# RocketFlash/EmbeddingNet

Measured on AMD Instinct MI355X. Metric: images/sec training (ResNet18, 224², triplet batch-hard) @ 1/2/4/8 GPU, higher is better.
Workload: dtype f32; 1 GPU; resnet18 224x224x3 synthetic U[0,1), 107-class P x K sampling, local batch 32x4=128 (139 resident batches cycled), E=256, margin 0.5, mining 'hardest' per local batch, radam, fp32 tensors (conv products on 16-bit MFMA from operand splits, fp32 accumulate: 3x3 stride-1 convs and their weight gradients, and the ResNets' other convs where both operands' ranges are known: two fp16 pieces + a per-tenso; global_batch=128, parallelism=dp1, active_triplets_min=192, dead_steps=0, resident_batches=139, step_mode=eager, mining=hardest

## Files before the change

### embeddingnet_amd/csrc/nn_kernels.hip

```cpp
#include "common.h"
#include "multi_tensor.h"
#include "gemm_engine.h"
#include <stdlib.h>
#include "../../include/embnet.h"

namespace embnet {

__device__ __forceinline__ float4 ld4(const float* p, long i) { return reinterpret_cast<const float4*>(p)[i]; }
__device__ __forceinline__ void st4(float* p, long i, float4 v) { reinterpret_cast<float4*>(p)[i] = v; }
__device__ __forceinline__ void add4(float4& a, float4 v) { a.x += v.x; a.y += v.y; a.z += v.z; a.w += v.w; }
__device__ __forceinline__ float4 affine4(float4 v, float4 sc, float4 sh) {
  return make_float4(fmaf(v.x, sc.x, sh.x), fmaf(v.y, sc.y, sh.y), fmaf(v.z, sc.z, sh.z), fmaf(v.w, sc.w, sh.w));
}
__device__ __forceinline__ float4 act_apply4(int act, float4 v) {
  return make_float4(act_apply(act, v.x), act_apply(act, v.y), act_apply(act, v.z), act_apply(act, v.w));
}
__device__ __forceinline__ float4 act_grad4(int act, float4 xv, float4 sc, float4 sh, float4 dz) {
  return make_float4(act_grad(act, fmaf(xv.x, sc.x, sh.x), dz.x), act_grad(act, fmaf(xv.y, sc.y, sh.y), dz.y),
                     act_grad(act, fmaf(xv.z, sc.z, sh.z), dz.z), act_grad(act, fmaf(xv.w, sc.w, sh.w), dz.w));
}
__device__ __forceinline__ float4 relu_mask4(float4 x, float4 v) {
  return make_float4(x.x > 0.f ? v.x : 0.f, x.y > 0.f ? v.y : 0.f, x.z > 0.f ? v.z : 0.f, x.w > 0.f ? v.w : 0.f);
}

// ... 30 lines not shown
  DropArg d{seed, seed_add, 0u, 1.f};
  if (rate > 0.f) { d.thr = (uint32_t)((double)rate * 4294967296.0); d.keep_scale = 1.f / (1.f - rate); }
  return d;
}
static DropArg no_drop() { return drop_arg(0.f, 0, nullptr); }
__device__ __forceinline__ uint64_t drop_seed(const DropArg& d) { return d.seed + (d.seed_add ? *d.seed_add : 0ull); }
__device__ __forceinline__ float4 drop4(const DropArg& d, uint64_t seed, long i4, float4 v) {
  const uint64_t e = (uint64_t)i4 * 4;
  v.x = rng_u32(seed, e, 1) >= d.thr ? v.x * d.keep_scale : 0.f;
  v.y = rng_u32(seed, e + 1, 1) >= d.thr ? v.y * d.keep_scale : 0.f;
  v.z = rng_u32(seed, e + 2, 1) >= d.thr ? v.z * d.keep_scale : 0.f;
  v.w = rng_u32(seed, e + 3, 1) >= d.thr ? v.w * d.keep_scale : 0.f;
  return v;
}

struct ColGeom { int cl, rl, blocks, rows_per_block; };

static ColGeom col_geom(long m, int c) {
  ColGeom g;
  int cl = 1; while (cl < c && cl < 256) cl <<= 1;
  g.cl = cl; g.rl = 256 / cl;
  long blocks = (m + (long)g.rl * 16 - 1) / ((long)g.rl * 16);
  if (blocks < 512) {
    blocks = (m + (long)g.rl * 4 - 1) / ((long)g.rl * 4);
    if (blocks > 512) blocks = 512;
  }
  if (blocks > 2048) blocks = 2048;
  if (blocks < 1) blocks = 1;
  g.blocks = (int)blocks;
  g.rows_per_block = (int)((m + blocks - 1) / blocks);
  return g;
}

template <class F>
__device__ __forceinline__ void col_reduce2(long m, int c, ColGeom g, float* __restrict__ partial, F f) {
  __shared__ float sh[2][256];
  const int ci = threadIdx.x % g.cl, ri = threadIdx.x / g.cl;
  const long r0 = (long)blockIdx.x * g.rows_per_block;
  const long r1 = min(r0 + g.rows_per_block, m);
  for (int c0 = 0; c0 < c; c0 += g.cl) {
    const int col = c0 + ci;
    float a = 0.f, b = 0.f;
    if (col < c)
      for (long r = r0 + ri; r < r1; r += g.rl) f(r, col, a, b);
    sh[0][threadIdx.x] = a; sh[1][threadIdx.x] = b;
// ... 49 lines not shown
}
__device__ __forceinline__ float tensor_bound(const float* __restrict__ bound, int c) {
  float m = 0.f;
  for (int i = threadIdx.x; i < c; i += 256) m = fmaxf(m, bound[i]);
  return block_max256<true>(m);
}

__global__ __launch_bounds__(256) void bn_stats_kernel(const float* __restrict__ x, long m, int c, ColGeom g,
                                                       float* __restrict__ partial) {
  col_reduce2(m, c, g, partial, [&](long r, int col, float& a, float& b) {
    const float v = x[r * c + col]; a += v; b = fmaf(v, v, b);
  });
}

struct NoPrep { __device__ __forceinline__ int operator()(int) const { return 0; } };
template <bool MAX3 = false, class P, class F>
__device__ __forceinline__ void col_reduce2_v4p(long m, int c4, ColGeom g, float* __restrict__ partial, P prep, F f,
                                                float* __restrict__ pmax = nullptr) {
  __shared__ float4 sh4[MAX3 ? 3 : 2][256];
  const int ci = threadIdx.x % g.cl, ri = threadIdx.x / g.cl;
  const long r0 = (long)blockIdx.x * g.rows_per_block;
  const long r1 = min(r0 + g.rows_per_block, m);
  for (int q0 = 0; q0 < c4; q0 += g.cl) {
    const int q = q0 + ci;
    float4 a = make_float4(0.f, 0.f, 0.f, 0.f), b = a, mx = a;
    if (q < c4) {
      const auto k = prep(q);
      long r = r0 + ri;
      const long rl = g.rl;
      if constexpr (MAX3) {
        for (; r + 3 * rl < r1; r += 4 * rl) { f(r, q, k, a, b, mx); f(r + rl, q, k, a, b, mx); f(r + 2 * rl, q, k, a, b, mx); f(r + 3 * rl, q, k, a, b, mx); }
        for (; r < r1; r += rl) f(r, q, k, a, b, mx);
      } else {
        for (; r + 3 * rl < r1; r += 4 * rl) { f(r, q, k, a, b); f(r + rl, q, k, a, b); f(r + 2 * rl, q, k, a, b); f(r + 3 * rl, q, k, a, b); }
        for (; r < r1; r += rl) f(r, q, k, a, b);
      }
    }
    int groups = g.rl;
    if (g.cl < 64) {
      for (int o = g.cl; o < 64; o <<= 1) {
        a.x += __shfl_xor(a.x, o, 64); a.y += __shfl_xor(a.y, o, 64); a.z += __shfl_xor(a.z, o, 64); a.w += __shfl_xor(a.w, o, 64);
        b.x += __shfl_xor(b.x, o, 64); b.y += __shfl_xor(b.y, o, 64); b.z += __shfl_xor(b.z, o, 64); b.w += __shfl_xor(b.w, o, 64);
        if constexpr (MAX3) {
          mx.x = fmaxf(mx.x, __shfl_xor(mx.x, o, 64)); mx.y = fmaxf(mx.y, __shfl_xor(mx.y, o, 64));
          mx.z = fmaxf(mx.z, __shfl_xor(mx.z, o, 64)); mx.w = fmaxf(mx.w, __shfl_xor(mx.w, o, 64));
        }
      }
      groups = 4;
      if ((threadIdx.x & 63) < g.cl) {
        sh4[0][(threadIdx.x >> 6) * g.cl + ci] = a; sh4[1][(threadIdx.x >> 6) * g.cl + ci] = b;
        if constexpr (MAX3) sh4[2][(threadIdx.x >> 6) * g.cl + ci] = mx;
      }
    } else {
      sh4[0][threadIdx.x] = a; sh4[1][threadIdx.x] = b;
      if constexpr (MAX3) sh4[2][threadIdx.x] = mx;
    }
    __syncthreads();
    if (ri == 0 && q < c4) {
      a = sh4[0][ci]; b = sh4[1][ci];
      if constexpr (MAX3) mx = sh4[2][ci];
      for (int k = 1; k < groups; ++k) {
        const float4 oa = sh4[0][k * g.cl + ci], ob = sh4[1][k * g.cl + ci];
        add4(a, oa); add4(b, ob);
        if constexpr (MAX3) {
          const float4 om = sh4[2][k * g.cl + ci];
          mx.x = fmaxf(mx.x, om.x); mx.y = fmaxf(mx.y, om.y); mx.z = fmaxf(mx.z, om.z); mx.w = fmaxf(mx.w, om.w);
        }
      }
      st4(partial + ((long)blockIdx.x * 2 + 0) * c4 * 4, q, a);
      st4(partial + ((long)blockIdx.x * 2 + 1) * c4 * 4, q, b);
      if constexpr (MAX3) st4(pmax + (long)blockIdx.x * c4 * 4, q, mx);
    }
    __syncthreads();
  }
}
template <class F>
__device__ __forceinline__ void col_reduce2_v4(long m, int c4, ColGeom g, float* __restrict__ partial, F f) {
  col_reduce2_v4p(m, c4, g, partial, NoPrep(), [&](long r, int q, int, float4& a, float4& b) { f(r, q, a, b); });
}

__global__ __launch_bounds__(256) void bn_stats4_kernel(const float* __restrict__ x, long m, int c4, ColGeom g,
                                                        float* __restrict__ partial) {
  col_reduce2_v4(m, c4, g, partial, [&](long r, int q, float4& a, float4& b) {
    const float4 v = ld4(x, r * c4 + q);
    add4(a, v);
    b.x = fmaf(v.x, v.x, b.x); b.y = fmaf(v.y, v.y, b.y); b.z = fmaf(v.z, v.z, b.z); b.w = fmaf(v.w, v.w, b.w);
  });
}

__device__ __forceinline__ float4 ld_pad4(const float* __restrict__ x, long p, int c, int q) {
  const float* s = x + p * c + 4 * q;
  if (c == 3) return make_float4(s[0], s[1], s[2], 0.f);
  const int live = c - 4 * q;
  return make_float4(s[0], live > 1 ? s[1] : 0.f, live > 2 ? s[2] : 0.f, live > 3 ? s[3] : 0.f);
}
__global__ __launch_bounds__(256) void bn_stats_pad4_kernel(const float* __restrict__ x, long m, int c, int c4, ColGeom g,
                                                            float* __restrict__ partial) {
  col_reduce2_v4(m, c4, g, partial, [&](long r, int q, float4& a, float4& b) {
    const float4 v = ld_pad4(x, r, c, q);
    add4(a, v);
    b.x = fmaf(v.x, v.x, b.x); b.y = fmaf(v.y, v.y, b.y); b.z = fmaf(v.z, v.z, b.z); b.w = fmaf(v.w, v.w, b.w);
  });
}

__global__ __launch_bounds__(256) void bn_bwd_reduce4_kernel(const float* __restrict__ dy, const float* __restrict__ x,
                                                             long m, int c4, ColGeom g, const float* __restrict__ mean,
                                                             const float* __restrict__ rstd, const float* __restrict__ scale,
                                                             const float* __restrict__ shift, int relu,
                                                             float* __restrict__ partial, const DropArg drop, float* __restrict__ pmax) {
  const uint64_t dseed = drop.thr ? drop_seed(drop) : 0ull;
  auto prep = [&](int q) { return bn_consts<false>(q, scale, shift, mean, rstd, nullptr, nullptr, 1); };
  auto body = [&](long r, int q, const BnConsts& k, float4& a, float4& b, float4& mx) {
    const float4 xv = ld4(x, r * c4 + q);
    float4 dz = ld4(dy, r * c4 + q);
    if (drop.thr) dz = drop4(drop, dseed, r * c4 + q, dz);
    if (relu) dz = act_grad4(relu, xv, k.sc, k.sh, dz);
    bn_sums4(a, b, dz, xv, k.mu, k.rs);
    mx.x = fmaxf(mx.x, fabsf(dz.x)); mx.y = fmaxf(mx.y, fabsf(dz.y)); mx.z = fmaxf(mx.z, fabsf(dz.z)); mx.w = fmaxf(mx.w, fabsf(dz.w));
  };
  if (pmax) col_reduce2_v4p<true>(m, c4, g, partial, prep, body, pmax);
  else col_reduce2_v4p(m, c4, g, partial, prep, [&](long r, int q, const BnConsts& k, float4& a, float4& b) {
    float4 mx = make_float4(0.f, 0.f, 0.f, 0.f); body(r, q, k, a, b, mx);
  });
}

template <int MODE, class DZ>
__device__ __forceinline__ void bn_bwd_apply4_body(DZ dz_of, const float* __restrict__ x, long total4, int c4, float inv_m,
                                                   const float* __restrict__ mean, const float* __restrict__ rstd,
                                                   const float* __restrict__ scale, const float* __restrict__ shift,
                                                   const float* __restrict__ dbeta, const float* __restrict__ dgamma, int relu,
                                                   int training, const float* __restrict__ dx_add, float* __restrict__ dx,
                                                   unsigned short* __restrict__ dx_planes, uint32_t* __restrict__ range_slot,
                                                   const float* __restrict__ dx_bound, const uint32_t* __restrict__ add_range) {
  const long stride = (long)gridDim.x * 256;
  const bool fixed = stride % c4 == 0;
  const float4 z4 = make_float4(0.f, 0.f, 0.f, 0.f);
  BnConsts k{z4, z4, z4, z4, z4, z4};
// ... 75 lines not shown
                     __fadd_rn(__fmul_rn(g.z, inv), dy.z), __fadd_rn(__fmul_rn(g.w, inv), dy.w));
}
__device__ __forceinline__ float4 gate4(float4 dy, const float* __restrict__ gate, long idx) {
  if (!gate) return dy;
  const float4 s = ld4(gate, idx);
  return make_float4(__fmul_rn(dy.x, s.x), __fmul_rn(dy.y, s.y), __fmul_rn(dy.z, s.z), __fmul_rn(dy.w, s.w));
}

__global__ __launch_bounds__(256) void bn_bwd_reduce4_gap_kernel(const float* __restrict__ dy, const float* __restrict__ dpool,
                                                                 const float* __restrict__ gate, DivU dhw, float inv_hw, const float* __restrict__ x, long m,
                                                                 int c4, ColGeom g, const float* __restrict__ mean,
                                                                 const float* __restrict__ rstd, const float* __restrict__ scale,
                                                                 const float* __restrict__ shift, int relu,
                                                                 float* __restrict__ partial) {
  col_reduce2_v4p(m, c4, g, partial, [&](int q) { return bn_consts<false>(q, scale, shift, mean, rstd, nullptr, nullptr, 1); },
                  [&](long r, int q, const BnConsts& k, float4& a, float4& b) {
    const float4 xv = ld4(x, r * c4 + q);
    const long nq = (long)divu((uint32_t)r, dhw) * c4 + q;
    const float4 gp = ld4(dpool, nq);
    float4 dz = add_pool4(gate4(ld4(dy, r * c4 + q), gate, nq), gp, inv_hw);
    if (relu) dz = act_grad4(relu, xv, k.sc, k.sh, dz);
    bn_sums4(a, b, dz, xv, k.mu, k.rs);
  });
}

__global__ __launch_bounds__(256) void bn_bwd_apply4_gap_kernel(const float* __restrict__ dy, const float* __restrict__ dpool,
                                                                const float* __restrict__ gate, DivU dhwc4, float inv_hw, const float* __restrict__ x,
                                                                long total4, int c4, float inv_m, const float* __restrict__ mean,
                                                                const float* __restrict__ rstd, const float* __restrict__ scale,
                                                                const float* __restrict__ shift, const float* __restrict__ dbeta,
                                                                const float* __restrict__ dgamma, int relu, float* __restrict__ dx) {
  bn_bwd_apply4_body<0>([&](long i) {
    const long nq = (long)divu((uint32_t)i, dhwc4) * c4 + (int)(i % c4);
    const float4 gp = ld4(dpool, nq);
    return add_pool4(gate4(ld4(dy, i), gate, nq), gp, inv_hw);
// ... 89 lines not shown
  b = wave_sum(b); g = wave_sum(g);
  if (lane == 0) { dbeta[col] = (float)b; dgamma[col] = (float)g; }
}

__global__ __launch_bounds__(256) void bn_bwd_apply_inrelu4_kernel(const float* __restrict__ dy, const float* __restrict__ x,
                                                                   long m, int c4, ColGeom g, float inv_m,
                                                                   const float* __restrict__ mean, const float* __restrict__ rstd,
                                                                   const float* __restrict__ scale, const float* __restrict__ shift,
                                                                   const float* __restrict__ dbeta, const float* __restrict__ dgamma,
                                                                   int relu, int training, float* __restrict__ dz_out,
                                                                   float* __restrict__ partial, const DropArg drop,
                                                                   uint32_t* __restrict__ range_slot) {
  const uint64_t dseed = drop.thr ? drop_seed(drop) : 0ull;
  float amax = 0.f;
  col_reduce2_v4p(m, c4, g, partial, [&](int q) { return bn_consts(q, scale, shift, mean, rstd, dbeta, dgamma, training); },
                  [&](long r, int q, const BnConsts& k, float4& a, float4&) {
    const float4 xv = ld4(x, r * c4 + q);
    float4 dz = ld4(dy, r * c4 + q);
    if (drop.thr) dz = drop4(drop, dseed, r * c4 + q, dz);
    if (relu) dz = act_grad4(relu, xv, k.sc, k.sh, dz);
    const float4 o = relu_mask4(xv, bn_dx4(dz, xv, k, inv_m, training));
    reinterpret_cast<float4*>(dz_out)[r * c4 + q] = o;
    add4(a, o);
    amax = amax4(amax, o);
  });
  if (range_slot) range_emit_block(range_slot + 1 + blockIdx.x % RANGE_PARTIALS, amax);
}

__global__ __launch_bounds__(256) void bn_finalize_kernel(const float* __restrict__ partial, int blocks, long m, int c,
                                                          const float* __restrict__ gamma, const float* __restrict__ beta,
                                                          float eps, float momentum, float* __restrict__ mean_out,
                                                          float* __restrict__ rstd_out, float* __restrict__ scale,
                                                          float* __restrict__ shift, float* __restrict__ moving_mean,
// ... 292 lines not shown
  const long i = (long)blockIdx.x * 256 + threadIdx.x;
  if (i >= total) return;
  const int col = (int)(i % c4);
  long t = i / c4;
  const int iw = (int)(t % w); t /= w;
  const int ih = (int)(t % h);
  const int b = (int)(t / h);
  st4(dx, i, pool_taps_grad4(dy, argmax, b, ih, iw, col, c4, k, stride, pad, oh, ow));
}

__global__ __launch_bounds__(256) void maxpool_relu_bwd_colsum4_kernel(
    const float* __restrict__ dy, const uint8_t* __restrict__ argmax, const float* __restrict__ y, long m, int h, int w,
    DivU dw, DivU dh, int c4, int k, int stride, int pad, int oh, int ow, ColGeom g, float* __restrict__ dz,
    float* __restrict__ partial, uint32_t* __restrict__ range_slot) {
  float amax = 0.f;
  col_reduce2_v4(m, c4, g, partial, [&](long r, int q, float4& a, float4& b) {
    const uint32_t t = divu((uint32_t)r, dw);
    const int iw = (int)((uint32_t)r - t * (uint32_t)w);
    const uint32_t img = divu(t, dh);
    const int ih = (int)(t - img * (uint32_t)h);
    const float4 v = relu_mask4(ld4(y, r * c4 + q), pool_taps_grad4(dy, argmax, (int)img, ih, iw, q, c4, k, stride, pad, oh, ow));
    st4(dz, r * c4 + q, v);
    add4(a, v);
    amax = amax4(amax, v);
  });
  if (range_slot) range_emit_block(range_slot + 1 + blockIdx.x % RANGE_PARTIALS, amax);
}

__global__ __launch_bounds__(256) void affine_act_maxpool_fwd4_kernel(
    const float* __restrict__ x, int n, int h, int w, int c4, const float* __restrict__ scale,
    const float* __restrict__ shift, int act, int k, int stride, int pad, int oh, int ow, float* __restrict__ y,
    uint8_t* __restrict__ argmax, float* __restrict__ xwin) {
  const long total = (long)n * oh * ow * c4;
  const long i = (long)blockIdx.x * 256 + threadIdx.x;
  if (i >= total) return;
  const int col = (int)(i % c4);
// ... 2 lines not shown
  const int y_o = (int)(t % oh);
  const int b = (int)(t / oh);
  const float4 sc = ld4(scale, col), sh = ld4(shift, col);
  const PoolWin win = pool_scan4(x, b, y_o, x_o, h, w, col, c4, k, stride, pad,
                                 [&](float4 v) { return act_apply4(act, affine4(v, sc, sh)); });
  if (xwin) st4(xwin, i, make_float4(win.xin[0], win.xin[1], win.xin[2], win.xin[3]));
  st4(y, i, make_float4(win.best[0], win.best[1], win.best[2], win.best[3]));
  reinterpret_cast<uint32_t*>(argmax)[i] = pack_taps(win.tap);
}

__global__ __launch_bounds__(256) void pool_bn_bwd_reduce4_kernel(
    const float* __restrict__ dy, const uint8_t* __restrict__ argmax, const float* __restrict__ x, long mp, int h, int w,
    int c4, int k, int stride, int pad, int oh, int ow, ColGeom g, const float* __restrict__ mean,
    const float* __restrict__ rstd, const float* __restrict__ scale, const float* __restrict__ shift, int act,
    const float* __restrict__ xwin, float* __restrict__ partial) {
  col_reduce2_v4(mp, c4, g, partial, [&](long r, int q, float4& a, float4& b) {
    const uint32_t am = reinterpret_cast<const uint32_t*>(argmax)[r * c4 + q];
    float4 xw4 = make_float4(0.f, 0.f, 0.f, 0.f);
    if (xwin) xw4 = ld4(xwin, r * c4 + q);
    const float xwv[4] = {xw4.x, xw4.y, xw4.z, xw4.w};
    const float4 d = ld4(dy, r * c4 + q);
    const int x_o = (int)(r % ow); const long t = r / ow;
    const int y_o = (int)(t % oh), bb = (int)(t / oh);
    const float4 sc = ld4(scale, q), sh = ld4(shift, q), mu = ld4(mean, q), rs = ld4(rstd, q);
    const float dd[4] = {d.x, d.y, d.z, d.w}, scv[4] = {sc.x, sc.y, sc.z, sc.w}, shv[4] = {sh.x, sh.y, sh.z, sh.w};
    const float muv[4] = {mu.x, mu.y, mu.z, mu.w}, rsv[4] = {rs.x, rs.y, rs.z, rs.w};
    float av[4], bv[4];
#pragma unroll
    for (int j = 0; j < 4; ++j) {
      const uint32_t tap = (am >> (8 * j)) & 0xff;
      const bool on = tap != 255u;
      const uint32_t tp = on ? tap : 0u;
      const int ih = min(max(y_o * stride - pad + (int)(tp / (uint32_t)k), 0), h - 1);
      const int iw = min(max(x_o * stride - pad + (int)(tp % (uint32_t)k), 0), w - 1);
      const float xv = xwin ? xwv[j] : x[((((long)bb * h + ih) * w + iw) * c4 + q) * 4 + j];
      const float dz = on ? act_grad(act, fmaf(xv, scv[j], shv[j]), dd[j]) : 0.f;
// ... 436 lines not shown
                             float* y_bound, uint32_t* y_range, void* stream, float* xhat_bound = nullptr) {
  EMBNET_CHECK_ARG(x && save_mean && save_rstd && scale && shift && workspace, "bn_train_fwd: null pointer");
  EMBNET_CHECK_ARG(m > 0 && c > 0, "bn_train_fwd: m=%ld c=%d", m, c);
  EMBNET_CHECK_ARG(!y_range || (y_bound && y && !(reinterpret_cast<uintptr_t>(y_range) & 3)),
                   "bn_train_fwd: y_range (the range slot of the fp32 y) goes with y_bound and y");
  if (const int e = bn_workspace_check("bn_train_fwd", workspace_bytes, m, c)) return e;
  const ColGeom g = col_geom(m, c);
  const float* partial = (const float*)workspace;
  int nblocks = g.blocks;
  if (partial_in) {
    EMBNET_CHECK_ARG(partial_rows > 0, "bn_train_fwd: partial_rows=%d", partial_rows);
    partial = partial_in; nblocks = partial_rows;
  } else if ((c & 3) == 0) {
    const ColGeom g4 = col_geom(m, c / 4);
    nblocks = g4.blocks;
    { EMBNET_TRACE("embnet::bn_stats4_kernel", TRACE_BYTES, 4.0 * m * c, stream); bn_stats4_kernel<<<g4.blocks, 256, 0, S(stream)>>>(x, m, c / 4, g4, (float*)workspace); }
  } else {
    { EMBNET_TRACE("embnet::bn_stats_kernel", TRACE_BYTES, 4.0 * m * c, stream); bn_stats_kernel<<<g.blocks, 256, 0, S(stream)>>>(x, m, c, g, (float*)workspace); }
  }
  { EMBNET_TRACE("embnet::bn_finalize_kernel", TRACE_BYTES, 8.0 * nblocks * c, stream); bn_finalize_kernel<<<c, 256, 0, S(stream)>>>(partial, nblocks, m, c, gamma, beta, eps, momentum, save_mean,
                                                          save_rstd, scale, shift, moving_mean, moving_var, partial_in != nullptr, y_bound, xhat_bound); }
  if (y)
    launch_affine_act(x, m, c, scale, shift, relu, y, no_drop(), y_bound, y_range, stream);
  return check_launch("bn_train_fwd");
}
extern "C" int embnet_bn_train_fwd(const float* x, long m, int c, const float* gamma, const float* beta, float eps,
                                   float momentum, int relu, float* y, float* save_mean, float* save_rstd,
                                   float* scale, float* shift, float* moving_mean, float* moving_var,
                                   const float* partial_in, int partial_rows, void* workspace, size_t workspace_bytes,
                                   void* stream) {
  return bn_train_fwd_impl(x, m, c, gamma, beta, eps, momentum, relu, y, save_mean, save_rstd, scale, shift, moving_mean, moving_var,
// ... 7 lines not shown
  return bn_train_fwd_impl(x, m, c, gamma, beta, eps, momentum, relu, y, save_mean, save_rstd, scale, shift, moving_mean, moving_var,
                           partial_in, partial_rows, workspace, workspace_bytes, y_bound, y_range, stream, xhat_bound);
}

extern "C" int embnet_bn_train_fwd_pad_ex(const float* x, long m, int c, int cp, const float* gamma, const float* beta, float eps,
                                          float momentum, int act, float* y, float* save_mean, float* save_rstd, float* scale,
                                          float* shift, float* moving_mean, float* moving_var, void* workspace,
                                          size_t workspace_bytes, float* y_bound, uint32_t* y_range, float* xhat_bound, void* stream) {
  EMBNET_CHECK_ARG(x && y && save_mean && save_rstd && scale && shift && workspace, "bn_train_fwd_pad: null pointer");
  EMBNET_CHECK_ARG(m > 0 && c > 0 && (c & 3) && cp == (c + 3) / 4 * 4, "bn_train_fwd_pad: m=%ld c=%d cp=%d", m, c, cp);
  EMBNET_CHECK_ARG(!y_range || (y_bound && !(reinterpret_cast<uintptr_t>(y_range) & 3)),
                   "bn_train_fwd_pad: y_range (the range slot of y) goes with y_bound");
  if (const int e = bn_workspace_check("bn_train_fwd_pad", workspace_bytes, m, cp)) return e;
  const int c4 = cp / 4;
  const ColGeom g4 = col_geom(m, c4);
  { EMBNET_TRACE("embnet::bn_stats_pad4_kernel", TRACE_BYTES, 4.0 * m * c, stream); bn_stats_pad4_kernel<<<g4.blocks, 256, 0, S(stream)>>>(x, m, c, c4, g4, (float*)workspace); }
  { EMBNET_TRACE("embnet::bn_finalize_kernel", TRACE_BYTES, 8.0 * g4.blocks * cp, stream); bn_finalize_kernel<<<cp, 256, 0, S(stream)>>>((const float*)workspace, g4.blocks, m, cp, gamma, beta, eps, momentum, save_mean,
                                                          save_rstd, scale, shift, moving_mean, moving_var, 0, y_bound, xhat_bound); }
  { EMBNET_TRACE("embnet::pad_affine_act_kernel", TRACE_BYTES, 4.0 * m * (c + cp), stream); pad_affine_act_kernel<<<ew_blocks_c4(m * c4, c4), 256, 0, S(stream)>>>(x, m * c4, c, c4, scale, shift, act, y, y_bound, y_range); }
  return check_launch("bn_train_fwd_pad");
}

extern "C" int embnet_bn_infer_fwd(const float* x, long m, int c, const float* gamma, const float* beta,
                                   const float* moving_mean, const float* moving_var, float eps, int relu, float* y,
                                   float* scale, float* shift, void* stream) {
  EMBNET_CHECK_ARG(x && moving_mean && moving_var && scale && shift, "bn_infer_fwd: null pointer");
  EMBNET_CHECK_ARG(m > 0 && c > 0, "bn_infer_fwd: m=%ld c=%d", m, c);
  bn_infer_prepare_kernel<<<cdiv(c, 256), 256, 0, S(stream)>>>(c, gamma, beta, moving_mean, moving_var, eps, scale, shift);
  if (y) launch_affine_act(x, m, c, scale, shift, relu, y, no_drop(), nullptr, nullptr, stream);
  return check_launch("bn_infer_fwd");
}
// ... 115 lines not shown
  EMBNET_CHECK_ARG(dx || (c & 3) == 0, "bn_bwd: dx = NULL (planes only) needs the four-channel kernels");
  EMBNET_CHECK_ARG(!dx_planes || ((c & 15) == 0 && (size_t)m * c * 2 < 0x7FFFFFF0ull / 3), "bn_bwd: dx_planes needs c %% 16 == 0");
  EMBNET_CHECK_ARG(!training || (save_mean && save_rstd), "bn_bwd: training needs saved statistics");
  EMBNET_CHECK_ARG(m > 0 && c > 0, "bn_bwd: m=%ld c=%d", m, c);
  if (const int e = bn_workspace_check("bn_bwd", workspace_bytes, m, c)) return e;
  const ColGeom g = col_geom(m, c);
  float* partial = (float*)workspace;
  const bool bound = dx_planes && planes_f16() && (c & 3) == 0 && save_mean && save_rstd &&
                     (xhat_bound || !training) && (!dx_add || dx_add_range);
  float* dx_bound = nullptr;
  if (save_mean && save_rstd) {
    if ((c & 3) == 0) {
      const ColGeom g4 = col_geom(m, c / 4);
      float* pmax = bound ? partial + (size_t)g4.blocks * 2 * c : nullptr;
      if (bound) dx_bound = pmax + (size_t)g4.blocks * c;
      { EMBNET_TRACE("embnet::bn_bwd_reduce4_kernel", TRACE_BYTES, 8.0 * m * c, stream); bn_bwd_reduce4_kernel<<<g4.blocks, 256, 0, S(stream)>>>(dy, x, m, c / 4, g4, save_mean, save_rstd, scale, shift, relu, partial, no_drop(), pmax); }
      bn_bwd_finalize_kernel<<<c, 256, 0, S(stream)>>>(partial, g4.blocks, c, dbeta, dgamma, 0, bound ? nullptr : emit, pmax, scale, xhat_bound,
                                                       1.f / (float)m, training, dx_bound);
    } else {
      { EMBNET_TRACE("embnet::bn_bwd_reduce_kernel", TRACE_BYTES, 8.0 * m * c, stream); bn_bwd_reduce_kernel<<<g.blocks, 256, 0, S(stream)>>>(dy, x, m, c, g, save_mean, save_rstd, scale, shift, relu, partial); }
      bn_bwd_finalize_kernel<<<c, 256, 0, S(stream)>>>(partial, g.blocks, c, dbeta, dgamma);
    }
  } else {
    zero2_kernel<<<cdiv(c, 256), 256, 0, S(stream)>>>(dbeta, dgamma, c);
  }
  if ((c & 3) == 0)
    launch_bn_bwd_apply4(dy, x, m, c, save_mean, save_rstd, scale, shift, dbeta, dgamma, relu, training, dx_add, dx, dx_planes, S(stream), emit, dx_bound, dx_add_range);
  else
    { EMBNET_TRACE("embnet::bn_bwd_apply_kernel", TRACE_BYTES, (dx_add ? 16.0 : 12.0) * m * c, stream); bn_bwd_apply_kernel<<<ew_blocks(m * c), 256, 0, S(stream)>>>(dy, x, m * c, c, 1.f / (float)m, save_mean, save_rstd,
                                                                 scale, shift, dbeta, dgamma, relu, training, dx_add, dx); }
  return check_launch("bn_bwd");
// ... 25 lines not shown
  EMBNET_CHECK_ARG(!(reinterpret_cast<uintptr_t>(slot) & 3), what ": the range slot is 4-byte aligned")

static int bn_bwd_inrelu_impl(const float* dy, const float* x, long m, int c, const float* save_mean,
                              const float* save_rstd, const float* scale, const float* shift, int relu, int training,
                              float* dz, float* dgamma, float* dbeta, float* dbias, void* workspace,
                              size_t workspace_bytes, void* stream, const DropArg drop, uint32_t* dz_range = nullptr) {
  EMBNET_CHECK_ARG(!take_emit_slot(), "bn_bwd_inrelu: the deprecated embnet_range_emit request is not served here: pass dz_range to the _ex form");
  EMBNET_RANGE_ARG(dz_range, "bn_bwd_inrelu");
  EMBNET_CHECK_ARG(dy && x && scale && shift && dz && dgamma && dbeta && dbias && workspace, "bn_bwd_inrelu: null pointer");
  EMBNET_CHECK_ARG(m > 0 && c > 0 && (c & 3) == 0, "bn_bwd_inrelu: m=%ld c=%d (c %% 4 == 0 required)", m, c);
  EMBNET_CHECK_ARG(!training || (save_mean && save_rstd), "bn_bwd_inrelu: training needs saved statistics");
  if (const int e = bn_workspace_check("bn_bwd_inrelu", workspace_bytes, m, c)) return e;
  float* partial = (float*)workspace;
  const ColGeom g4 = col_geom(m, c / 4);
  if (save_mean && save_rstd) {
    { EMBNET_TRACE("embnet::bn_bwd_reduce4_kernel", TRACE_BYTES, 8.0 * m * c, stream); bn_bwd_reduce4_kernel<<<g4.blocks, 256, 0, S(stream)>>>(dy, x, m, c / 4, g4, save_mean, save_rstd, scale, shift, relu, partial, drop, nullptr); }
    bn_bwd_finalize_kernel<<<c, 256, 0, S(stream)>>>(partial, g4.blocks, c, dbeta, dgamma, 0, dz_range);
  } else {
    zero2_kernel<<<cdiv(c, 256), 256, 0, S(stream)>>>(dbeta, dgamma, c);
    range_begin(dz_range, stream);
  }
  { EMBNET_TRACE("embnet::bn_bwd_apply_inrelu4_kernel", TRACE_BYTES, 12.0 * m * c, stream);
    bn_bwd_apply_inrelu4_kernel<<<g4.blocks, 256, 0, S(stream)>>>(dy, x, m, c / 4, g4, 1.f / (float)m, save_mean, save_rstd, scale, shift,
                                                               dbeta, dgamma, relu, training, dz, partial, drop, dz_range); }
  colsum_finalize_kernel<<<c, 256, 0, S(stream)>>>(partial, g4.blocks, c, dbias, dz_range);
  return check_launch("bn_bwd_inrelu");
}

extern "C" int embnet_bn_bwd_gap(const float* dy, const float* dpool, const float* gate, int n, int hw, const float* x, int c, const float* save_mean,
                                 const float* save_rstd, const float* scale, const float* shift, int relu, float* dx,
                                 float* dgamma, float* dbeta, void* workspace, size_t workspace_bytes, void* stream) {
  EMBNET_CHECK_ARG(!take_emit_slot(), "bn_bwd_gap: this pass cannot emit the range requested by embnet_range_emit");
  EMBNET_CHECK_ARG(dy && dpool && x && save_mean && save_rstd && scale && shift && dx && dgamma && dbeta && workspace, "bn_bwd_gap: null pointer");
  EMBNET_CHECK_ARG(n > 0 && hw > 0 && c > 0 && (c & 3) == 0, "bn_bwd_gap: n=%d hw=%d c=%d (c %% 4 == 0)", n, hw, c);
  const long m = (long)n * hw;
  EMBNET_CHECK_ARG(m * (c / 4) < 0x7FFFFFFFl, "bn_bwd_gap: tensor too large");
  if (const int e = bn_workspace_check("bn_bwd_gap", workspace_bytes, m, c)) return e;
  float* partial = (float*)workspace;
  const ColGeom g4 = col_geom(m, c / 4);
  const float inv_hw = 1.f / (float)hw;
  { EMBNET_TRACE("embnet::bn_bwd_reduce4_gap_kernel", TRACE_BYTES, 8.0 * m * c, stream);
    bn_bwd_reduce4_gap_kernel<<<g4.blocks, 256, 0, S(stream)>>>(dy, dpool, gate, make_divu((uint32_t)hw), inv_hw, x, m, c / 4, g4, save_mean, save_rstd,
                                                                scale, shift, relu, partial); }
  bn_bwd_finalize_kernel<<<c, 256, 0, S(stream)>>>(partial, g4.blocks, c, dbeta, dgamma);
  { EMBNET_TRACE("embnet::bn_bwd_apply4_gap_kernel", TRACE_BYTES, 12.0 * m * c, stream);
    bn_bwd_apply4_gap_kernel<<<ew_blocks_c4(m * c / 4, c / 4), 256, 0, S(stream)>>>(dy, dpool, gate, make_divu((uint32_t)((long)hw * (c / 4))), inv_hw, x,
                                                                                    m * c / 4, c / 4, 1.f / (float)m, save_mean, save_rstd,
                                                                                    scale, shift, dbeta, dgamma, relu, dx); }
  return check_launch("bn_bwd_gap");
}

extern "C" int embnet_se_bn_sums(const float* dg, const float* x, int n, int hw, int c, const float* save_mean, const float* save_rstd,
                                 const float* scale, const float* shift, int act, float* sums, void* stream) {
  EMBNET_CHECK_ARG(dg && x && save_mean && save_rstd && scale && shift && sums, "se_bn_sums: null pointer");
  EMBNET_CHECK_ARG(n > 0 && hw > 0 && c > 0 && (c & 3) == 0 && act >= 0 && act <= 2, "se_bn_sums: n=%d hw=%d c=%d act=%d (c %% 4 == 0)", n, hw, c, act);
  EMBNET_TRACE("embnet::se_bn_sums4_kernel", TRACE_BYTES, 8.0 * n * hw * c, stream);
  const PixGeom g = pix_geom(n, hw, c / 4);
// ... 127 lines not shown
                                                 int c, int k, int stride, int pad, int oh, int ow, float* dz, float* dbias,
                                                 void* workspace, size_t workspace_bytes, uint32_t* dz_range, void* stream) {
  EMBNET_CHECK_ARG(dy && argmax && y && dz && dbias && workspace, "maxpool_relu_bwd_colsum: null pointer");
  EMBNET_RANGE_ARG(dz_range, "maxpool_relu_bwd_colsum");
  EMBNET_CHECK_ARG(n > 0 && h > 0 && w > 0 && c > 0 && k > 0 && stride > 0 && oh > 0 && ow > 0 && pad >= 0,
                   "maxpool_relu_bwd_colsum: bad geometry");
  EMBNET_CHECK_ARG((c & 3) == 0, "maxpool_relu_bwd_colsum: channel count %d not a multiple of 4 (use maxpool_bwd + relu_bwd_colsum)", c);
  EMBNET_CHECK_ARG((oh - 1) * stride + k <= h + 2 * pad && (ow - 1) * stride + k <= w + 2 * pad,
                   "maxpool_relu_bwd_colsum: window leaves the padded image");
  const long m = (long)n * h * w;
  EMBNET_CHECK_ARG(m < (1l << 31), "maxpool_relu_bwd_colsum: %ld pixels (limit 2^31 - 1)", m);
  if (const int e = bn_workspace_check("maxpool_relu_bwd_colsum", workspace_bytes, m, c)) return e;
  const ColGeom g4 = col_geom(m, c / 4);
  range_begin(dz_range, stream);
  { EMBNET_TRACE("embnet::maxpool_relu_bwd_colsum4_kernel", TRACE_BYTES, 8.0 * m * c + 5.0 * n * oh * ow * c, stream);
    maxpool_relu_bwd_colsum4_kernel<<<g4.blocks, 256, 0, S(stream)>>>(dy, argmax, y, m, h, w, make_divu((uint32_t)w), make_divu((uint32_t)h),
                                                                       c / 4, k, stride, pad, oh, ow, g4, dz, (float*)workspace, dz_range); }
  colsum_finalize_kernel<<<c, 256, 0, S(stream)>>>((const float*)workspace, g4.blocks, c, dbias, dz_range);
  return check_launch("maxpool_relu_bwd_colsum");
}
extern "C" int embnet_maxpool_relu_bwd_colsum(const float* dy, const uint8_t* argmax, const float* y, int n, int h, int w,
                                              int c, int k, int stride, int pad, int oh, int ow, float* dz, float* dbias,
                                              void* workspace, size_t workspace_bytes, void* stream) {
  return embnet_maxpool_relu_bwd_colsum_ex(dy, argmax, y, n, h, w, c, k, stride, pad, oh, ow, dz, dbias, workspace, workspace_bytes,
                                           nullptr, stream);
}

extern "C" int embnet_bn_act_maxpool_fwd(const float* x, int n, int h, int w, int c, const float* scale, const float* shift,
                                         int act, int k, int stride, int pad, int oh, int ow, float* y, uint8_t* argmax,
                                         float* xwin, void* stream) {
  EMBNET_CHECK_ARG(x && scale && shift && y && argmax, "bn_act_maxpool_fwd: null pointer");
// ... 15 lines not shown
static int bn_act_maxpool_bwd_impl(const float* dy, const uint8_t* argmax, const float* x, int n, int h, int w, int c,
                                   int k, int stride, int pad, int oh, int ow, const float* save_mean,
                                   const float* save_rstd, const float* scale, const float* shift, int act,
                                   int training, const float* xwin, float* dx, float* dgamma, float* dbeta,
                                   void* workspace, size_t workspace_bytes, uint32_t* emit, void* stream, int band_rows = 0) {
  EMBNET_CHECK_ARG(!emit || (save_mean && save_rstd && !(reinterpret_cast<uintptr_t>(emit) & 3)),
                   "bn_act_maxpool_bwd: a range of dx was requested without saved statistics (or the slot is not 4-byte aligned)");
  EMBNET_CHECK_ARG(dy && argmax && x && scale && shift && dx && dgamma && dbeta && workspace, "bn_act_maxpool_bwd: null pointer");
  EMBNET_CHECK_ARG(!training || (save_mean && save_rstd), "bn_act_maxpool_bwd: training needs saved statistics");
  EMBNET_CHECK_ARG(n > 0 && h > 0 && w > 0 && c > 0 && k > 0 && stride > 0 && oh > 0 && ow > 0, "bn_act_maxpool_bwd: bad geometry");
  EMBNET_CHECK_ARG((c & 3) == 0, "bn_act_maxpool_bwd: channel count %d not a multiple of 4", c);
  const long mp = (long)n * oh * ow;
  if (const int e = bn_workspace_check("bn_act_maxpool_bwd", workspace_bytes, mp, c)) return e;
  if (save_mean && save_rstd) {
    const ColGeom g4 = col_geom(mp, c / 4);
    { EMBNET_TRACE("embnet::pool_bn_bwd_reduce4_kernel", TRACE_BYTES, 9.0 * mp * c, stream); pool_bn_bwd_reduce4_kernel<<<g4.blocks, 256, 0, S(stream)>>>(dy, argmax, x, mp, h, w, c / 4, k, stride, pad, oh, ow, g4,
                                                                 save_mean, save_rstd, scale, shift, act, xwin, (float*)workspace); }
    bn_bwd_finalize_kernel<<<c, 256, 0, S(stream)>>>((const float*)workspace, g4.blocks, c, dbeta, dgamma, 0, emit);
  } else {
    zero2_kernel<<<cdiv(c, 256), 256, 0, S(stream)>>>(dbeta, dgamma, c);
  }
  const long total = (long)n * h * w * (c / 4);
  if (band_rows > 0) {
    const long rows = (long)n * h, w4 = (long)w * (c / 4), segs = cdiv(w4, 256), bands = cdiv(rows, band_rows);
    EMBNET_CHECK_ARG(w4 < (1l << 31) - 256 && segs * bands < (1l << 31), "bn_act_maxpool_bwd: %ld x %ld workgroups", segs, bands);
    EMBNET_TRACE("embnet::pool_bn_bwd_apply_band4_kernel", TRACE_BYTES, 32.0 * total + 5.0 * mp * c, stream);
    pool_bn_bwd_apply_band4_kernel<<<(unsigned)(segs * bands), 256, 0, S(stream)>>>(dy, argmax, x, rows, h, w, c / 4, k, stride, pad, oh, ow,
                                                                                   (int)segs, band_rows, 1.f / (float)((long)n * h * w),
                                                                                   save_mean, save_rstd, scale, shift, dbeta, dgamma, act,
                                                                                   training, dx, emit);
  } else
// ... 302 lines not shown
```

Before: 16780 images/sec.

## Make BN column reductions persistent with software-prefetched row loads

The column-reduction helper now launches a grid capped at four workgroups per compute unit, and each workgroup loops over several row bands, writing per-band partials so the finalize kernels stay unchanged. Loads are split into a separate fetch lambda that prefetches the next four rows into registers while the current ones are accumulated, with double-buffered shared memory between bands. This targets wave-launch overhead and exposed memory latency in the BN statistics and backward reduction kernels. In exchange it uses more registers and shared memory, which can lower occupancy, and the tail handling for bands under four rows is more complex.

Result: no change. 16890 images/sec, median of 6 (+0.6%).

```diff
diff --git a/embeddingnet_amd/csrc/nn_kernels.hip b/embeddingnet_amd/csrc/nn_kernels.hip
--- a/embeddingnet_amd/csrc/nn_kernels.hip
+++ b/embeddingnet_amd/csrc/nn_kernels.hip
@@ -68,7 +68,18 @@
   return v;
 }
 
-struct ColGeom { int cl, rl, blocks, rows_per_block; };
+struct ColGeom { int cl, rl, blocks, rows_per_block, grid; };
+constexpr int COL_WG_PER_CU = 4;
+
+static int compute_units() {
+  static const int n = [] {
+    int dev = 0, cus = 0;
+    if (hipGetDevice(&dev) == hipSuccess && hipDeviceGetAttribute(&cus, hipDeviceAttributeMultiprocessorCount, dev) == hipSuccess && cus > 0)
+      return cus;
+    return 256;
+  }();
+  return n;
+}
 
 static ColGeom col_geom(long m, int c) {
   ColGeom g;
@@ -83,6 +94,8 @@
   if (blocks < 1) blocks = 1;
   g.blocks = (int)blocks;
   g.rows_per_block = (int)((m + blocks - 1) / blocks);
+  const long grid = (long)COL_WG_PER_CU * compute_units();
+  g.grid = (int)(blocks < grid ? blocks : grid);
   return g;
 }
 
@@ -162,75 +175,100 @@
 }
 
 struct NoPrep { __device__ __forceinline__ int operator()(int) const { return 0; } };
-template <bool MAX3 = false, class P, class F>
-__device__ __forceinline__ void col_reduce2_v4p(long m, int c4, ColGeom g, float* __restrict__ partial, P prep, F f,
+template <bool MAX3 = false, class P, class L, class F>
+__device__ __forceinline__ void col_reduce2_v4p(long m, int c4, ColGeom g, float* __restrict__ partial, P prep, L ld, F f,
                                                 float* __restrict__ pmax = nullptr) {
-  __shared__ float4 sh4[MAX3 ? 3 : 2][256];
+  __shared__ float4 sh4buf[2][MAX3 ? 3 : 2][256];
+  using D = decltype(ld(0L, 0));
   const int ci = threadIdx.x % g.cl, ri = threadIdx.x / g.cl;
-  const long r0 = (long)blockIdx.x * g.rows_per_block;
-  const long r1 = min(r0 + g.rows_per_block, m);
+  const long rl = g.rl;
+  auto acc = [&](long r, int q, const auto& k, const D& d, float4& a, float4& b, float4& mx) {
+    if constexpr (MAX3) f(r, q, k, d, a, b, mx); else f(r, q, k, d, a, b);
+  };
+  int par = 0;
   for (int q0 = 0; q0 < c4; q0 += g.cl) {
     const int q = q0 + ci;
-    float4 a = make_float4(0.f, 0.f, 0.f, 0.f), b = a, mx = a;
-    if (q < c4) {
-      const auto k = prep(q);
-      long r = r0 + ri;
-      const long rl = g.rl;
-      if constexpr (MAX3) {
-        for (; r + 3 * rl < r1; r += 4 * rl) { f(r, q, k, a, b, mx); f(r + rl, q, k, a, b, mx); f(r + 2 * rl, q, k, a, b, mx); f(r + 3 * rl, q, k, a, b, mx); }
-        for (; r < r1; r += rl) f(r, q, k, a, b, mx);
+    const bool live = q < c4;
+    const auto k = prep(live ? q : 0);
+    long band = blockIdx.x;
+    long r = band * g.rows_per_block + ri, r1 = min((band + 1) * g.rows_per_block, m);
+    D d[4];
+    auto fetch = [&] {
+      if (!live || band >= g.blocks) return;
+      if (r + 3 * rl < r1) {
+        d[0] = ld(r, q); d[1] = ld(r + rl, q); d[2] = ld(r + 2 * rl, q); d[3] = ld(r + 3 * rl, q);
       } else {
-        for (; r + 3 * rl < r1; r += 4 * rl) { f(r, q, k, a, b); f(r + rl, q, k, a, b); f(r + 2 * rl, q, k, a, b); f(r + 3 * rl, q, k, a, b); }
-        for (; r < r1; r += rl) f(r, q, k, a, b);
+#pragma unroll
+        for (int j = 0; j < 3; ++j) if (r + j * rl < r1) d[j] = ld(r + j * rl, q);
       }
-    }
-    int groups = g.rl;
-    if (g.cl < 64) {
-      for (int o = g.cl; o < 64; o <<= 1) {
-        a.x += __shfl_xor(a.x, o, 64); a.y += __shfl_xor(a.y, o, 64); a.z += __shfl_xor(a.z, o, 64); a.w += __shfl_xor(a.w, o, 64);
-        b.x += __shfl_xor(b.x, o, 64); b.y += __shfl_xor(b.y, o, 64); b.z += __shfl_xor(b.z, o, 64); b.w += __shfl_xor(b.w, o, 64);
-        if constexpr (MAX3) {
-          mx.x = fmaxf(mx.x, __shfl_xor(mx.x, o, 64)); mx.y = fmaxf(mx.y, __shfl_xor(mx.y, o, 64));
-          mx.z = fmaxf(mx.z, __shfl_xor(mx.z, o, 64)); mx.w = fmaxf(mx.w, __shfl_xor(mx.w, o, 64));
+    };
+    fetch();
+    for (; band < g.blocks; par ^= 1) {
+      float4 (*sh4)[256] = sh4buf[par];
+      float4 a = make_float4(0.f, 0.f, 0.f, 0.f), b = a, mx = a;
+      const long done = band;
+      while (band == done) {
+        if (live) {
+          if (r + 3 * rl < r1) {
+            acc(r, q, k, d[0], a, b, mx); acc(r + rl, q, k, d[1], a, b, mx); acc(r + 2 * rl, q, k, d[2], a, b, mx); acc(r + 3 * rl, q, k, d[3], a, b, mx);
+          } else {
+#pragma unroll
+            for (int j = 0; j < 3; ++j) if (r + j * rl < r1) acc(r + j * rl, q, k, d[j], a, b, mx);
+          }
         }
+        r += 4 * rl;
+        if (r - ri >= r1) {
+          band += gridDim.x;
+          r = band * g.rows_per_block + ri; r1 = min((band + 1) * g.rows_per_block, m);
+        }
+        fetch();
       }
-      groups = 4;
-      if ((threadIdx.x & 63) < g.cl) {
-        sh4[0][(threadIdx.x >> 6) * g.cl + ci] = a; sh4[1][(threadIdx.x >> 6) * g.cl + ci] = b;
-        if constexpr (MAX3) sh4[2][(threadIdx.x >> 6) * g.cl + ci] = mx;
+      int groups = g.rl;
+      if (g.cl < 64) {
+        for (int o = g.cl; o < 64; o <<= 1) {
+          a.x += __shfl_xor(a.x, o, 64); a.y += __shfl_xor(a.y, o, 64); a.z += __shfl_xor(a.z, o, 64); a.w += __shfl_xor(a.w, o, 64);
+          b.x += __shfl_xor(b.x, o, 64); b.y += __shfl_xor(b.y, o, 64); b.z += __shfl_xor(b.z, o, 64); b.w += __shfl_xor(b.w, o, 64);
+          if constexpr (MAX3) {
+            mx.x = fmaxf(mx.x, __shfl_xor(mx.x, o, 64)); mx.y = fmaxf(mx.y, __shfl_xor(mx.y, o, 64));
+            mx.z = fmaxf(mx.z, __shfl_xor(mx.z, o, 64)); mx.w = fmaxf(mx.w, __shfl_xor(mx.w, o, 64));
+          }
+        }
+        groups = 4;
+        if ((threadIdx.x & 63) < g.cl) {
+          sh4[0][(threadIdx.x >> 6) * g.cl + ci] = a; sh4[1][(threadIdx.x >> 6) * g.cl + ci] = b;
+          if constexpr (MAX3) sh4[2][(threadIdx.x >> 6) * g.cl + ci] = mx;
+        }
+      } else {
+        sh4[0][threadIdx.x] = a; sh4[1][threadIdx.x] = b;
+        if constexpr (MAX3) sh4[2][threadIdx.x] = mx;
       }
-    } else {
-      sh4[0][threadIdx.x] = a; sh4[1][threadIdx.x] = b;
-      if constexpr (MAX3) sh4[2][threadIdx.x] = mx;
-    }
-    __syncthreads();
-    if (ri == 0 && q < c4) {
-      a = sh4[0][ci]; b = sh4[1][ci];
-      if constexpr (MAX3) mx = sh4[2][ci];
-      for (int k = 1; k < groups; ++k) {
-        const float4 oa = sh4[0][k * g.cl + ci], ob = sh4[1][k * g.cl + ci];
-        add4(a, oa); add4(b, ob);
-        if constexpr (MAX3) {
-          const float4 om = sh4[2][k * g.cl + ci];
-          mx.x = fmaxf(mx.x, om.x); mx.y = fmaxf(mx.y, om.y); mx.z = fmaxf(mx.z, om.z); mx.w = fmaxf(mx.w, om.w);
+      __syncthreads();
+      if (ri == 0 && q < c4) {
+        a = sh4[0][ci]; b = sh4[1][ci];
+        if constexpr (MAX3) mx = sh4[2][ci];
+        for (int w = 1; w < groups; ++w) {
+          const float4 oa = sh4[0][w * g.cl + ci], ob = sh4[1][w * g.cl + ci];
+          add4(a, oa); add4(b, ob);
+          if constexpr (MAX3) {
+            const float4 om = sh4[2][w * g.cl + ci];
+            mx.x = fmaxf(mx.x, om.x); mx.y = fmaxf(mx.y, om.y); mx.z = fmaxf(mx.z, om.z); mx.w = fmaxf(mx.w, om.w);
+          }
         }
+        st4(partial + (done * 2 + 0) * c4 * 4, q, a);
+        st4(partial + (done * 2 + 1) * c4 * 4, q, b);
+        if constexpr (MAX3) st4(pmax + done * c4 * 4, q, mx);
       }
-      st4(partial + ((long)blockIdx.x * 2 + 0) * c4 * 4, q, a);
-      st4(partial + ((long)blockIdx.x * 2 + 1) * c4 * 4, q, b);
-      if constexpr (MAX3) st4(pmax + (long)blockIdx.x * c4 * 4, q, mx);
-    }
-    __syncthreads();
-  }
-}
-template <class F>
-__device__ __forceinline__ void col_reduce2_v4(long m, int c4, ColGeom g, float* __restrict__ partial, F f) {
-  col_reduce2_v4p(m, c4, g, partial, NoPrep(), [&](long r, int q, int, float4& a, float4& b) { f(r, q, a, b); });
+    }
+  }
+}
+template <class L, class F>
+__device__ __forceinline__ void col_reduce2_v4(long m, int c4, ColGeom g, float* __restrict__ partial, L ld, F f) {
+  col_reduce2_v4p(m, c4, g, partial, NoPrep(), ld, [&](long r, int q, int, const auto& d, float4& a, float4& b) { f(r, q, d, a, b); });
 }
 
 __global__ __launch_bounds__(256) void bn_stats4_kernel(const float* __restrict__ x, long m, int c4, ColGeom g,
                                                         float* __restrict__ partial) {
-  col_reduce2_v4(m, c4, g, partial, [&](long r, int q, float4& a, float4& b) {
-    const float4 v = ld4(x, r * c4 + q);
+  col_reduce2_v4(m, c4, g, partial, [&](long r, int q) { return ld4(x, r * c4 + q); }, [&](long, int, float4 v, float4& a, float4& b) {
     add4(a, v);
     b.x = fmaf(v.x, v.x, b.x); b.y = fmaf(v.y, v.y, b.y); b.z = fmaf(v.z, v.z, b.z); b.w = fmaf(v.w, v.w, b.w);
   });
@@ -244,13 +282,13 @@
 }
 __global__ __launch_bounds__(256) void bn_stats_pad4_kernel(const float* __restrict__ x, long m, int c, int c4, ColGeom g,
                                                             float* __restrict__ partial) {
-  col_reduce2_v4(m, c4, g, partial, [&](long r, int q, float4& a, float4& b) {
-    const float4 v = ld_pad4(x, r, c, q);
+  col_reduce2_v4(m, c4, g, partial, [&](long r, int q) { return ld_pad4(x, r, c, q); }, [&](long, int, float4 v, float4& a, float4& b) {
     add4(a, v);
     b.x = fmaf(v.x, v.x, b.x); b.y = fmaf(v.y, v.y, b.y); b.z = fmaf(v.z, v.z, b.z); b.w = fmaf(v.w, v.w, b.w);
   });
 }
 
+struct XDy { float4 x, dy; };
 __global__ __launch_bounds__(256) void bn_bwd_reduce4_kernel(const float* __restrict__ dy, const float* __restrict__ x,
                                                              long m, int c4, ColGeom g, const float* __restrict__ mean,
                                                              const float* __restrict__ rstd, const float* __restrict__ scale,
@@ -258,17 +296,18 @@
                                                              float* __restrict__ partial, const DropArg drop, float* __restrict__ pmax) {
   const uint64_t dseed = drop.thr ? drop_seed(drop) : 0ull;
   auto prep = [&](int q) { return bn_consts<false>(q, scale, shift, mean, rstd, nullptr, nullptr, 1); };
-  auto body = [&](long r, int q, const BnConsts& k, float4& a, float4& b, float4& mx) {
-    const float4 xv = ld4(x, r * c4 + q);
-    float4 dz = ld4(dy, r * c4 + q);
+  auto ld = [&](long r, int q) { return XDy{ld4(x, r * c4 + q), ld4(dy, r * c4 + q)}; };
+  auto body = [&](long r, int q, const BnConsts& k, const XDy& d, float4& a, float4& b, float4& mx) {
+    const float4 xv = d.x;
+    float4 dz = d.dy;
     if (drop.thr) dz = drop4(drop, dseed, r * c4 + q, dz);
     if (relu) dz = act_grad4(relu, xv, k.sc, k.sh, dz);
     bn_sums4(a, b, dz, xv, k.mu, k.rs);
     mx.x = fmaxf(mx.x, fabsf(dz.x)); mx.y = fmaxf(mx.y, fabsf(dz.y)); mx.z = fmaxf(mx.z, fabsf(dz.z)); mx.w = fmaxf(mx.w, fabsf(dz.w));
   };
-  if (pmax) col_reduce2_v4p<true>(m, c4, g, partial, prep, body, pmax);
-  else col_reduce2_v4p(m, c4, g, partial, prep, [&](long r, int q, const BnConsts& k, float4& a, float4& b) {
-    float4 mx = make_float4(0.f, 0.f, 0.f, 0.f); body(r, q, k, a, b, mx);
+  if (pmax) col_reduce2_v4p<true>(m, c4, g, partial, prep, ld, body, pmax);
+  else col_reduce2_v4p(m, c4, g, partial, prep, ld, [&](long r, int q, const BnConsts& k, const XDy& d, float4& a, float4& b) {
+    float4 mx = make_float4(0.f, 0.f, 0.f, 0.f); body(r, q, k, d, a, b, mx);
   });
 }
 
@@ -374,11 +413,14 @@
                                                                  const float* __restrict__ shift, int relu,
                                                                  float* __restrict__ partial) {
   col_reduce2_v4p(m, c4, g, partial, [&](int q) { return bn_consts<false>(q, scale, shift, mean, rstd, nullptr, nullptr, 1); },
-                  [&](long r, int q, const BnConsts& k, float4& a, float4& b) {
-    const float4 xv = ld4(x, r * c4 + q);
+                  [&](long r, int q) {
     const long nq = (long)divu((uint32_t)r, dhw) * c4 + q;
     const float4 gp = ld4(dpool, nq);
-    float4 dz = add_pool4(gate4(ld4(dy, r * c4 + q), gate, nq), gp, inv_hw);
+    return XDy{ld4(x, r * c4 + q), add_pool4(gate4(ld4(dy, r * c4 + q), gate, nq), gp, inv_hw)};
+  },
+                  [&](long r, int q, const BnConsts& k, const XDy& d, float4& a, float4& b) {
+    const float4 xv = d.x;
+    float4 dz = d.dy;
     if (relu) dz = act_grad4(relu, xv, k.sc, k.sh, dz);
     bn_sums4(a, b, dz, xv, k.mu, k.rs);
   });
@@ -498,9 +540,10 @@
   const uint64_t dseed = drop.thr ? drop_seed(drop) : 0ull;
   float amax = 0.f;
   col_reduce2_v4p(m, c4, g, partial, [&](int q) { return bn_consts(q, scale, shift, mean, rstd, dbeta, dgamma, training); },
-                  [&](long r, int q, const BnConsts& k, float4& a, float4&) {
-    const float4 xv = ld4(x, r * c4 + q);
-    float4 dz = ld4(dy, r * c4 + q);
+                  [&](long r, int q) { return XDy{ld4(x, r * c4 + q), ld4(dy, r * c4 + q)}; },
+                  [&](long r, int q, const BnConsts& k, const XDy& d, float4& a, float4&) {
+    const float4 xv = d.x;
+    float4 dz = d.dy;
     if (drop.thr) dz = drop4(drop, dseed, r * c4 + q, dz);
     if (relu) dz = act_grad4(relu, xv, k.sc, k.sh, dz);
     const float4 o = relu_mask4(xv, bn_dx4(dz, xv, k, inv_m, training));
@@ -823,12 +866,13 @@
     DivU dw, DivU dh, int c4, int k, int stride, int pad, int oh, int ow, ColGeom g, float* __restrict__ dz,
     float* __restrict__ partial, uint32_t* __restrict__ range_slot) {
   float amax = 0.f;
-  col_reduce2_v4(m, c4, g, partial, [&](long r, int q, float4& a, float4& b) {
+  col_reduce2_v4(m, c4, g, partial, [&](long r, int q) {
     const uint32_t t = divu((uint32_t)r, dw);
     const int iw = (int)((uint32_t)r - t * (uint32_t)w);
     const uint32_t img = divu(t, dh);
     const int ih = (int)(t - img * (uint32_t)h);
-    const float4 v = relu_mask4(ld4(y, r * c4 + q), pool_taps_grad4(dy, argmax, (int)img, ih, iw, q, c4, k, stride, pad, oh, ow));
+    return relu_mask4(ld4(y, r * c4 + q), pool_taps_grad4(dy, argmax, (int)img, ih, iw, q, c4, k, stride, pad, oh, ow));
+  }, [&](long r, int q, float4 v, float4& a, float4& b) {
     st4(dz, r * c4 + q, v);
     add4(a, v);
     amax = amax4(amax, v);
@@ -861,12 +905,15 @@
     int c4, int k, int stride, int pad, int oh, int ow, ColGeom g, const float* __restrict__ mean,
     const float* __restrict__ rstd, const float* __restrict__ scale, const float* __restrict__ shift, int act,
     const float* __restrict__ xwin, float* __restrict__ partial) {
-  col_reduce2_v4(mp, c4, g, partial, [&](long r, int q, float4& a, float4& b) {
-    const uint32_t am = reinterpret_cast<const uint32_t*>(argmax)[r * c4 + q];
+  struct PoolIn { uint32_t am; float4 xw, dy; };
+  col_reduce2_v4(mp, c4, g, partial, [&](long r, int q) {
     float4 xw4 = make_float4(0.f, 0.f, 0.f, 0.f);
     if (xwin) xw4 = ld4(xwin, r * c4 + q);
-    const float xwv[4] = {xw4.x, xw4.y, xw4.z, xw4.w};
-    const float4 d = ld4(dy, r * c4 + q);
+    return PoolIn{reinterpret_cast<const uint32_t*>(argmax)[r * c4 + q], xw4, ld4(dy, r * c4 + q)};
+  }, [&](long r, int q, const PoolIn& in, float4& a, float4& b) {
+    const uint32_t am = in.am;
+    const float xwv[4] = {in.xw.x, in.xw.y, in.xw.z, in.xw.w};
+    const float4 d = in.dy;
     const int x_o = (int)(r % ow); const long t = r / ow;
     const int y_o = (int)(t % oh), bb = (int)(t / oh);
     const float4 sc = ld4(scale, q), sh = ld4(shift, q), mu = ld4(mean, q), rs = ld4(rstd, q);
@@ -1333,7 +1380,7 @@
   } else if ((c & 3) == 0) {
     const ColGeom g4 = col_geom(m, c / 4);
     nblocks = g4.blocks;
-    { EMBNET_TRACE("embnet::bn_stats4_kernel", TRACE_BYTES, 4.0 * m * c, stream); bn_stats4_kernel<<<g4.blocks, 256, 0, S(stream)>>>(x, m, c / 4, g4, (float*)workspace); }
+    { EMBNET_TRACE("embnet::bn_stats4_kernel", TRACE_BYTES, 4.0 * m * c, stream); bn_stats4_kernel<<<g4.grid, 256, 0, S(stream)>>>(x, m, c / 4, g4, (float*)workspace); }
   } else {
     { EMBNET_TRACE("embnet::bn_stats_kernel", TRACE_BYTES, 4.0 * m * c, stream); bn_stats_kernel<<<g.blocks, 256, 0, S(stream)>>>(x, m, c, g, (float*)workspace); }
   }
@@ -1371,7 +1418,7 @@
   if (const int e = bn_workspace_check("bn_train_fwd_pad", workspace_bytes, m, cp)) return e;
   const int c4 = cp / 4;
   const ColGeom g4 = col_geom(m, c4);
-  { EMBNET_TRACE("embnet::bn_stats_pad4_kernel", TRACE_BYTES, 4.0 * m * c, stream); bn_stats_pad4_kernel<<<g4.blocks, 256, 0, S(stream)>>>(x, m, c, c4, g4, (float*)workspace); }
+  { EMBNET_TRACE("embnet::bn_stats_pad4_kernel", TRACE_BYTES, 4.0 * m * c, stream); bn_stats_pad4_kernel<<<g4.grid, 256, 0, S(stream)>>>(x, m, c, c4, g4, (float*)workspace); }
   { EMBNET_TRACE("embnet::bn_finalize_kernel", TRACE_BYTES, 8.0 * g4.blocks * cp, stream); bn_finalize_kernel<<<cp, 256, 0, S(stream)>>>((const float*)workspace, g4.blocks, m, cp, gamma, beta, eps, momentum, save_mean,
                                                           save_rstd, scale, shift, moving_mean, moving_var, 0, y_bound, xhat_bound); }
   { EMBNET_TRACE("embnet::pad_affine_act_kernel", TRACE_BYTES, 4.0 * m * (c + cp), stream); pad_affine_act_kernel<<<ew_blocks_c4(m * c4, c4), 256, 0, S(stream)>>>(x, m * c4, c, c4, scale, shift, act, y, y_bound, y_range); }
@@ -1517,7 +1564,7 @@
       const ColGeom g4 = col_geom(m, c / 4);
       float* pmax = bound ? partial + (size_t)g4.blocks * 2 * c : nullptr;
       if (bound) dx_bound = pmax + (size_t)g4.blocks * c;
-      { EMBNET_TRACE("embnet::bn_bwd_reduce4_kernel", TRACE_BYTES, 8.0 * m * c, stream); bn_bwd_reduce4_kernel<<<g4.blocks, 256, 0, S(stream)>>>(dy, x, m, c / 4, g4, save_mean, save_rstd, scale, shift, relu, partial, no_drop(), pmax); }
+      { EMBNET_TRACE("embnet::bn_bwd_reduce4_kernel", TRACE_BYTES, 8.0 * m * c, stream); bn_bwd_reduce4_kernel<<<g4.grid, 256, 0, S(stream)>>>(dy, x, m, c / 4, g4, save_mean, save_rstd, scale, shift, relu, partial, no_drop(), pmax); }
       bn_bwd_finalize_kernel<<<c, 256, 0, S(stream)>>>(partial, g4.blocks, c, dbeta, dgamma, 0, bound ? nullptr : emit, pmax, scale, xhat_bound,
                                                        1.f / (float)m, training, dx_bound);
     } else {
@@ -1573,14 +1620,14 @@
   float* partial = (float*)workspace;
   const ColGeom g4 = col_geom(m, c / 4);
   if (save_mean && save_rstd) {
-    { EMBNET_TRACE("embnet::bn_bwd_reduce4_kernel", TRACE_BYTES, 8.0 * m * c, stream); bn_bwd_reduce4_kernel<<<g4.blocks, 256, 0, S(stream)>>>(dy, x, m, c / 4, g4, save_mean, save_rstd, scale, shift, relu, partial, drop, nullptr); }
+    { EMBNET_TRACE("embnet::bn_bwd_reduce4_kernel", TRACE_BYTES, 8.0 * m * c, stream); bn_bwd_reduce4_kernel<<<g4.grid, 256, 0, S(stream)>>>(dy, x, m, c / 4, g4, save_mean, save_rstd, scale, shift, relu, partial, drop, nullptr); }
     bn_bwd_finalize_kernel<<<c, 256, 0, S(stream)>>>(partial, g4.blocks, c, dbeta, dgamma, 0, dz_range);
   } else {
     zero2_kernel<<<cdiv(c, 256), 256, 0, S(stream)>>>(dbeta, dgamma, c);
     range_begin(dz_range, stream);
   }
   { EMBNET_TRACE("embnet::bn_bwd_apply_inrelu4_kernel", TRACE_BYTES, 12.0 * m * c, stream);
-    bn_bwd_apply_inrelu4_kernel<<<g4.blocks, 256, 0, S(stream)>>>(dy, x, m, c / 4, g4, 1.f / (float)m, save_mean, save_rstd, scale, shift,
+    bn_bwd_apply_inrelu4_kernel<<<g4.grid, 256, 0, S(stream)>>>(dy, x, m, c / 4, g4, 1.f / (float)m, save_mean, save_rstd, scale, shift,
                                                                dbeta, dgamma, relu, training, dz, partial, drop, dz_range); }
   colsum_finalize_kernel<<<c, 256, 0, S(stream)>>>(partial, g4.blocks, c, dbias, dz_range);
   return check_launch("bn_bwd_inrelu");
@@ -1599,7 +1646,7 @@
   const ColGeom g4 = col_geom(m, c / 4);
   const float inv_hw = 1.f / (float)hw;
   { EMBNET_TRACE("embnet::bn_bwd_reduce4_gap_kernel", TRACE_BYTES, 8.0 * m * c, stream);
-    bn_bwd_reduce4_gap_kernel<<<g4.blocks, 256, 0, S(stream)>>>(dy, dpool, gate, make_divu((uint32_t)hw), inv_hw, x, m, c / 4, g4, save_mean, save_rstd,
+    bn_bwd_reduce4_gap_kernel<<<g4.grid, 256, 0, S(stream)>>>(dy, dpool, gate, make_divu((uint32_t)hw), inv_hw, x, m, c / 4, g4, save_mean, save_rstd,
                                                                 scale, shift, relu, partial); }
   bn_bwd_finalize_kernel<<<c, 256, 0, S(stream)>>>(partial, g4.blocks, c, dbeta, dgamma);
   { EMBNET_TRACE("embnet::bn_bwd_apply4_gap_kernel", TRACE_BYTES, 12.0 * m * c, stream);
@@ -1757,7 +1804,7 @@
   const ColGeom g4 = col_geom(m, c / 4);
   range_begin(dz_range, stream);
   { EMBNET_TRACE("embnet::maxpool_relu_bwd_colsum4_kernel", TRACE_BYTES, 8.0 * m * c + 5.0 * n * oh * ow * c, stream);
-    maxpool_relu_bwd_colsum4_kernel<<<g4.blocks, 256, 0, S(stream)>>>(dy, argmax, y, m, h, w, make_divu((uint32_t)w), make_divu((uint32_t)h),
+    maxpool_relu_bwd_colsum4_kernel<<<g4.grid, 256, 0, S(stream)>>>(dy, argmax, y, m, h, w, make_divu((uint32_t)w), make_divu((uint32_t)h),
                                                                        c / 4, k, stride, pad, oh, ow, g4, dz, (float*)workspace, dz_range); }
   colsum_finalize_kernel<<<c, 256, 0, S(stream)>>>((const float*)workspace, g4.blocks, c, dbias, dz_range);
   return check_launch("maxpool_relu_bwd_colsum");
@@ -1803,7 +1850,7 @@
   if (const int e = bn_workspace_check("bn_act_maxpool_bwd", workspace_bytes, mp, c)) return e;
   if (save_mean && save_rstd) {
     const ColGeom g4 = col_geom(mp, c / 4);
-    { EMBNET_TRACE("embnet::pool_bn_bwd_reduce4_kernel", TRACE_BYTES, 9.0 * mp * c, stream); pool_bn_bwd_reduce4_kernel<<<g4.blocks, 256, 0, S(stream)>>>(dy, argmax, x, mp, h, w, c / 4, k, stride, pad, oh, ow, g4,
+    { EMBNET_TRACE("embnet::pool_bn_bwd_reduce4_kernel", TRACE_BYTES, 9.0 * mp * c, stream); pool_bn_bwd_reduce4_kernel<<<g4.grid, 256, 0, S(stream)>>>(dy, argmax, x, mp, h, w, c / 4, k, stride, pad, oh, ow, g4,
                                                                  save_mean, save_rstd, scale, shift, act, xwin, (float*)workspace); }
     bn_bwd_finalize_kernel<<<c, 256, 0, S(stream)>>>((const float*)workspace, g4.blocks, c, dbeta, dgamma, 0, emit);
   } else {
```
